# NeurAI-Lab/biHomE

Hardware: AMD Instinct MI355X
Metric: training image-pairs/s (128x128 patch, bs=64 per GPU, full step: fwd+bwd+Adam) (higher is better)
Workload: dtype f32

## Files before the change

bihome_amd/_lib.py:

```python
import ctypes
import os
from ctypes import POINTER, Structure, c_char_p, c_float, c_int, c_int64, c_void_p

_HERE = os.path.dirname(os.path.abspath(__file__))
TUNING = os.environ.get("BIHOME_TUNING") == "1"
_VARIANT = os.environ.get("BIHOME_LIB_VARIANT", "")
LIB_PATH = os.path.join(_HERE, "libbihome_hip_tuning.so" if TUNING else
                        ("libbihome_hip_%s.so" % _VARIANT if _VARIANT.isalnum() else "libbihome_hip.so"))


class BhConvDesc(Structure):
    _fields_ = [(n, c_int) for n in ("N", "Hi", "Wi", "Ci", "Ho", "Wo", "Co", "kh", "kw", "stride", "pad",
                                     "transposed", "in_nchw", "out_nchw", "precision", "w_layout", "route")] + \
               [("a_bound", c_void_p), ("b_bound", c_void_p)]


GEOMETRY_FIELDS = tuple(n for n, _ in BhConvDesc._fields_[:17])
AMAX_FLOATS = 512


class BhPack3x3Job(Structure):
    _fields_ = [("w", c_void_p), ("pf", c_void_p), ("pd", c_void_p), ("Co", c_int), ("Ci", c_int), ("split", c_int),
                ("reserved", c_int)]

# ... 117 lines not shown
        except AttributeError as e:
            raise BihomeLibError("bihome_amd: %s does not export %s (stale build?)" % (LIB_PATH, name)) from e
        fn.argtypes = argtypes
        fn.restype = c_int
    lib.bh_conv_wgrad_det_bytes.argtypes = [POINTER(BhConvDesc)]
    lib.bh_conv_wgrad_det_bytes.restype = c_int64
    lib.bh_stem7_wgrad_ws_bytes.argtypes = [POINTER(BhConvDesc)]
    lib.bh_stem7_wgrad_ws_bytes.restype = ctypes.c_size_t
    lib.bh_warp_bwd_img_scratch_doubles.argtypes = [c_int, c_int, c_int, c_int, c_int]
    lib.bh_warp_bwd_img_scratch_doubles.restype = ctypes.c_size_t
    if TUNING:
        lib.bh_debug_force_tile.argtypes = [c_int, c_int]
        lib.bh_debug_force_tile.restype = c_int
    return lib


lib = _load()
ROUTE_DETERMINISTIC, BN_DETERMINISTIC, F_DETERMINISTIC = 128, 32, 1
DSAC_METHODS = {"repr_error": 0, "inliers_ratio": 1, "soft_inliers_ratio": 2}
ROUTE_C3_PC = 512
ROUTE_WX3_PC = 1024
ROUTE_WX3_SHARED = 2048
ROUTE_GEMM_X3 = 4096
ROUTE_C3_TILE_WG = 256


def check(rc, what):
    if rc != 0:
        kind = {-1: "BH_E_BADARG", -2: "BH_E_UNSUPPORTED"}.get(rc, "hipError_t %d" % rc)
        raise BihomeLibError("%s failed: %s" % (what, kind))
```

bihome_amd/csrc/bn.hip:

```cpp
#include "common.h"

#define BN_MAX_CHUNKS 256

struct BnGeom {
    int groups, rows, C, C4, LPR, RPP, nchunks, rows_per_chunk;
    int det;
};

static bool bn_geom(int groups, int rows, int C, BnGeom& g, int det) {
    if (C % 4 || groups < 1 || rows < 1) return false;
    g.groups = groups; g.rows = rows; g.C = C; g.C4 = C / 4; g.det = det;
    if (g.C4 > 256 || (256 % g.C4)) return false;
    g.LPR = g.C4; g.RPP = 256 / g.LPR;
    int n = rows / (g.RPP * 4);
    if (n < 1) n = 1;
    if (n > BN_MAX_CHUNKS) n = BN_MAX_CHUNKS;
    g.rows_per_chunk = (rows + n - 1) / n;
    g.nchunks = (rows + g.rows_per_chunk - 1) / g.rows_per_chunk;
    return true;
}

template <int NV>
__device__ __forceinline__ void reduce_rows(double (&v)[NV], int LPR, int RPP, double* sm ) {
    for (int i = 0; i < NV; ++i) sm[threadIdx.x * NV + i] = v[i];
// ... 250 lines not shown
                                                           float* __restrict__ ggamma, float* __restrict__ gbeta,
                                                           unsigned* __restrict__ amax) {
    __shared__ float sm_amax[4];
    float vmax = 0.f;
    const int cq = threadIdx.x % g.LPR, r0 = threadIdx.x / g.LPR;
    const int grp = blockIdx.y;
    BnRaw raw[4];
    float4 cf4[4];
    double rs1[4], rs2[4];
#pragma unroll
    for (int i = 0; i < 4; ++i) {
        const int c = cq * 4 + i;
        cf4[i] = make_float4(0.f, 0.f, 0.f, 0.f); rs1[i] = 0; rs2[i] = 0;
        if (coef) {
            cf4[i] = coef[(size_t)grp * g.C + c];
            raw[i].gm = gamma ? gamma[c] : 1.f; raw[i].bt = beta ? beta[c] : 0.f; raw[i].s1 = 0; raw[i].s2 = 0;
        } else {
            raw[i] = bn_raw(stats, gamma, beta, nullptr, nullptr, 0, g.groups, grp, g.C, c, g.det);
            rs1[i] = bn_sum_total(sums, g.groups, grp, g.C, c, 0, g.det);
            rs2[i] = bn_sum_total(sums, g.groups, grp, g.C, c, 1, g.det);
        }
    }
    const size_t gbase = ((size_t)grp * g.rows) * g.C + cq * 4;
    const bool relu = flags & 1, mask_from_x = flags & 4;
    const bool rd_y = relu && !mask_from_x;
    const int stride = gridDim.x * g.RPP;
    int r = blockIdx.x * g.RPP + r0;
    float4 dv[4], av[4], yv[4];
    auto issue = [&](int rb) {
#pragma unroll
        for (int u = 0; u < 4; ++u) {
            const int rr = rb + u * stride;
            const size_t off = gbase + (size_t)rr * g.C;
            const bool ok = rr < g.rows;
            dv[u] = ok ? *reinterpret_cast<const float4*>(gy + off) : make_float4(0.f, 0.f, 0.f, 0.f);
            av[u] = ok ? *reinterpret_cast<const float4*>(x + off) : make_float4(0.f, 0.f, 0.f, 0.f);
            yv[u] = (ok && rd_y) ? *reinterpret_cast<const float4*>(y + off) : make_float4(0.f, 0.f, 0.f, 0.f);
        }
    };
    issue(r);
    float mean[4], invstd[4], sc[4], sh[4], k1[4], k2[4];
    const double inv_rows = 1.0 / (double)g.rows;
    const float invn = 1.0f / (float)g.rows;
#pragma unroll
    for (int i = 0; i < 4; ++i) {
        if (coef) {
            mean[i] = cf4[i].x; invstd[i] = cf4[i].y; k1[i] = cf4[i].z; k2[i] = cf4[i].w;
// ... 415 lines not shown
                       running_var, res, y, stats, g, eps, flags, use_running, momentum, upd ? running_mean : nullptr,
                       upd ? running_var : nullptr, reinterpret_cast<unsigned*>(amax_y));
    BH_LAUNCH_CHECK();
    return BH_OK;
}

int bh_bn_fwd_coeffs(const double* stats, const float* gamma, const float* beta, float* running_mean, float* running_var, int groups,
                     int rows, int C, float eps, float momentum, float* table, float* amax_y, void* stream) {
    BnGeom g;
    if (!stats || !table) return BH_E_BADARG;
    if (!bn_geom(groups, rows, C, g, -1)) return BH_E_UNSUPPORTED;
    const bool upd = running_mean && running_var;
    hipLaunchKernelGGL(bn_fwd_coeffs_kernel, dim3((groups * C + 255) / 256 + (upd ? 1 : 0)), dim3(256), 0, bh_stream(stream), stats, gamma, beta, g, eps,
                       momentum, upd ? running_mean : nullptr, upd ? running_var : nullptr, reinterpret_cast<float2*>(table),
                       reinterpret_cast<unsigned*>(amax_y));
    BH_LAUNCH_CHECK();
    return BH_OK;
}

int bh_bn_bwd(const float* gy, const float* y, const float* x, const float* gamma, const float* beta, const double* stats, float* gx,
              float* gres, float* ggamma, float* gbeta, double* scratch, int groups, int rows, int C, float eps, int flags,
              int use_running, const float* running_mean, const float* running_var, float* amax_gx, void* stream) {
    BnGeom g;
    if (!gy || !x || !gx || !stats || !scratch || ((flags & 1) && !(flags & 4) && !y)) return BH_E_BADARG;
    if ((flags & 4) && (flags & 2)) return BH_E_BADARG;
    if (C == 1) return amax_gx ? BH_E_UNSUPPORTED : bn1_bwd(gy, y, x, gamma, beta, stats, gx, gres, ggamma, gbeta, scratch, groups, rows, eps, flags, use_running,
                               running_mean, running_var, bh_stream(stream));
    if (!bn_geom(groups, rows, C, g, (flags & BH_BN_DETERMINISTIC) ? 1 : 0)) return BH_E_UNSUPPORTED;
    hipStream_t s = bh_stream(stream);
    if (flags & 16) {
        if (use_running) return BH_E_BADARG;
        hipLaunchKernelGGL(bn_bwd_apply_kernel, dim3(apply_blocks(g), groups), dim3(256), 0, s, gy, y, x, gamma, beta,
                           (const float4*)nullptr, gx, gres, g, flags, stats, (const double*)scratch, eps, ggamma, gbeta,
                           reinterpret_cast<unsigned*>(amax_gx));
        BH_LAUNCH_CHECK();
        return BH_OK;
    }
    float4* coef = reinterpret_cast<float4*>(scratch);
    double* part = scratch + (size_t)groups * C * 2;
    const bool need_sums = !use_running || ggamma || gbeta;
    if (need_sums) {
        hipLaunchKernelGGL(bn_bwd_reduce_kernel, dim3(g.nchunks, groups), dim3(256), 0, s, gy, y, x, gamma, beta, stats,
                           running_mean, running_var, g, eps, flags, use_running, part);
        BH_LAUNCH_CHECK();
    }
    BnGeom gf = g;
    if (!need_sums) gf.nchunks = 0;
    hipLaunchKernelGGL(bn_bwd_finalize_kernel, dim3(C), dim3(64), 0, s, part, gf, stats, running_mean, running_var, eps,
// ... 429 lines not shown
```

bihome_amd/csrc/conv3x3.hip:

```cpp
#include "common.h"
#include "conv3x3_args.h"
#include <type_traits>

#ifndef C3_X3_PIPE
#define C3_X3_PIPE 0
#endif

#ifndef C3_BN32_WAVES
#define C3_BN32_WAVES 2
#endif

#ifdef BH_TUNING
__device__ unsigned long long g_c3_ts[8 * 16384];
#define C3_STAMP(tile, k) do { if (a.dbg_ts && threadIdx.x == 0 && (tile) < 16384) { g_c3_ts[(tile) * 8 + (k)] = wall_clock64();          \
        if ((k) == 1 || (k) == 2) g_c3_ts[(tile) * 8 + 4 + (k)] = __builtin_readcyclecounter(); } } while (0)
#else
#define C3_STAMP(tile, k) do { } while (0)
#endif

constexpr int C3_HALO_BYTES = 8 * 200 * 16;
constexpr int C3_B_BYTES = 8192;
constexpr int C3_LDS_BYTES = 2 * C3_HALO_BYTES + 2 * C3_B_BYTES;

template <int BN, int SUBT, int TM, bool MAP4 = false>
// ... 77 lines not shown
#pragma unroll
                        for (int r = 0; r < 16; ++r)
                            zin[i][r] = __builtin_bit_cast(float, __builtin_amdgcn_raw_buffer_load_b32(rsZ, rowoff[r >> 2], C3_SOFF(i, r), 0));
                }
                if constexpr (ZM == 2) {
                    const __amdgpu_buffer_rsrc_t rsY = __builtin_amdgcn_make_buffer_rsrc(const_cast<float*>(a.bnr_y), 0, a.out_bytes, 0x00020000);
#pragma unroll
                    for (int i = 0; i < TM; ++i)
#pragma unroll
                        for (int r = 0; r < 16; ++r)
                            yin[i][r] = __builtin_bit_cast(float, __builtin_amdgcn_raw_buffer_load_b32(rsY, rowoff[r >> 2], C3_SOFF(i, r), 0));
                }
#pragma unroll
                for (int i = 0; i < TM; ++i)
#pragma unroll
                    for (int rq = 0; rq < 4; ++rq) {
                        float q1 = 0.f, q2 = 0.f;
#pragma unroll
                        for (int c = 0; c < 4; ++c) {
                            const int r = rq * 4 + c;
                            float v = acc[i][r] + bv;
                            if constexpr (HAS_EXTRA) v += ext[i][r];
                            if (a.relu) v = fmaxf(v, 0.0f);
                            __builtin_amdgcn_raw_buffer_store_b32(__builtin_bit_cast(unsigned, v), rsO, rowoff[rq], C3_SOFF(i, r), 0);
                            if constexpr (ZM > 0) {
                                const float zv = zin[i][r];
                                if (a.bnr_relu) {
                                    const float yv = ZM == 2 ? yin[i][r] : __builtin_fmaf(zv, r_sc, r_sh);
                                    if (!(yv > 0.f)) v = 0.f;
                                }
                                q1 += v; q2 = __builtin_fmaf(v, __builtin_fmaf(zv, r_invstd, c_x0), q2);
                            } else {
                                q1 += v; q2 = __builtin_fmaf(v, v, q2);
                            }
                        }
                        s1 += (double)q1; s2 += (double)q2;
                    }
            };
            using T_ = std::true_type; using F_ = std::false_type;
            using Z0 = std::integral_constant<int, 0>; using Z1 = std::integral_constant<int, 1>; using Z2 = std::integral_constant<int, 2>;
            if (rd_old || rd_res) {
                if (!rd_z) body(T_{}, Z0{}); else if (!rd_y) body(T_{}, Z1{}); else body(T_{}, Z2{});
            } else {
                if (!rd_z) body(F_{}, Z0{}); else if (!rd_y) body(F_{}, Z1{}); else body(F_{}, Z2{});
            }
        }
#undef C3_SOFF
    }
}

template <int BN, int PHASE>
__device__ __forceinline__ void c3_stats_merge(const C3Args& a, char* redb, double s1, double s2, int img, int g, int bx, int n0, int wave,
                                               int lane, int tid) {
    const int l31 = lane & 31, kh2 = lane >> 5;
    double* red = reinterpret_cast<double*>(redb);
// ... 552 lines not shown
                      d->Co % 64 == 0 && d->Ci % 64 == 0 && !bni && (!bn_sums || (groups >= 1 && d->N % groups == 0 && (d->N / groups) % 4 == 0));
    if (!map4 && (d->Hi % 8 || d->Wi % 8 || d->Ho != d->Hi || d->Wo != d->Wi)) return d->w_layout ? BH_E_UNSUPPORTED : 0;
    const int Kc = dgrad ? d->Co : d->Ci, Nn = dgrad ? d->Ci : d->Co;
    if (Kc % 32 || Nn % 32) return d->w_layout ? BH_E_UNSUPPORTED : 0;
    const int bn_tile = (Nn % 64) ? 32 : 64;
    const bool packed = d->w_layout != 0;
    const bool x3 = d->w_layout >= 2 && d->w_layout <= 4;
    const int np = d->w_layout >= 3 ? 2 : 3;
    const bool f16 = d->w_layout == 4;
    const bool bf16 = d->precision == 1;
    const long long src_bytes = (long long)d->N * d->Hi * d->Wi * Kc * 4, w_bytes = (long long)d->Co * 9 * d->Ci * (x3 ? 2 * np : 4);
    const long long out_bytes = (long long)d->N * d->Hi * d->Wi * Nn * 4;
    if (src_bytes >= (1ll << 31) || w_bytes >= (1ll << 31) || out_bytes >= (1ll << 31)) return 0;
    C3Args a = {};
    a.Src = src; a.Wt = w; a.bias = bias; a.Out = out;
    a.N = d->N; a.H = d->Hi; a.W = d->Wi; a.Kc = Kc; a.Nn = Nn; a.Cw = d->Ci; a.accumulate = accumulate;
    a.amax_src = reinterpret_cast<const unsigned*>(d->a_bound);
    a.src_bytes = (unsigned)src_bytes; a.w_bytes = (unsigned)w_bytes; a.out_bytes = (unsigned)out_bytes;
    if (bn_sums && (groups < 1 || d->N % groups || (!dgrad && bnr) || (dgrad && !bnr && accumulate))) return BH_E_BADARG;
    if (bnr) {
        if (!bnr->z || !bnr->stats) return BH_E_BADARG;
        a.bnr_z = bnr->z; a.bnr_y = bnr->y; a.bnr_stats = bnr->stats; a.bnr_gamma = bnr->gamma; a.bnr_beta = bnr->beta;
        a.bnr_eps = bnr->eps; a.bnr_relu = bnr->relu; a.bnr_rows = (d->N / groups) * d->Hi * d->Wi;
    }
    a.res = res; a.relu = relu; a.dbg_nch = g_c3_dbg_nch;
    a.bn_sums = bn_sums; a.imgs_per_group = bn_sums ? d->N / groups : 1; a.groups = groups;
    a.tiles_x = d->Wi / 8; a.tiles_per_img = (d->Hi / 8) * a.tiles_x; a.subtiles = d->N * a.tiles_per_img;
    if (map4) { a.tiles_x = 1; a.tiles_per_img = 1; a.subtiles = d->N / 4; }
    a.tx_shift = a.tpi_shift = -1;
    for (int b = 0; b < 24; ++b) {
        if (a.tiles_x == (1 << b)) a.tx_shift = b;
        if (a.tiles_per_img == (1 << b)) a.tpi_shift = b;
    }
    if (a.tx_shift < 0 || a.tpi_shift < 0) a.tx_shift = a.tpi_shift = -1;
    const bool few = (long long)((a.subtiles + 1) / 2) * (Nn / bn_tile) <= 256;
    const int subt = map4 ? 1 : (bn_tile == 64 && (g_c3_subt == 1 || (d->route & BH_ROUTE_C3_ONE_SUBTILE) || (g_c3_subt == 2 && few))) ? 1 : 2;
    dim3 grid((a.subtiles + subt - 1) / subt, Nn / bn_tile);
    a.gx_total = (int)grid.x; a.tpb = 1;
    {
        const long long wgs = (long long)grid.x * grid.y;
        if (g_c3_tpb >= 2 && !(d->route & BH_ROUTE_C3_ONE_POSITION) && subt == 2 && Kc / 32 > 1 && wgs > 512 && wgs <= 1024) {
            a.tpb = 2; grid.x = (grid.x + 1) / 2;
        }
    }
    if (bn_sums && !map4 && !(d->route & BH_ROUTE_C3_ONE_POSITION) && groups >= 1 && a.subtiles % (subt * groups) == 0) {
        const int ppg = a.subtiles / (subt * groups);
// ... 193 lines not shown
```

bihome_amd/csrc/conv3x3_args.h:

```cpp
#pragma once
#include "common.h"

typedef float f32x16 __attribute__((ext_vector_type(16)));
typedef float f32x8v __attribute__((ext_vector_type(8)));
typedef __bf16 bf16x8 __attribute__((ext_vector_type(8)));
typedef _Float16 f16x8 __attribute__((ext_vector_type(8)));
typedef __attribute__((address_space(3))) void* lds_void_ptr;

template <bool F16>
__device__ __forceinline__ f32x16 c3_mfma16(const uint4& av, const uint4& bv, const f32x16& c) {
    if constexpr (F16) return __builtin_amdgcn_mfma_f32_32x32x16_f16(__builtin_bit_cast(f16x8, av), __builtin_bit_cast(f16x8, bv), c, 0, 0, 0);
    else return __builtin_amdgcn_mfma_f32_32x32x16_bf16(__builtin_bit_cast(bf16x8, av), __builtin_bit_cast(bf16x8, bv), c, 0, 0, 0);
}

__device__ __forceinline__ bf16x8 c3_pack_bf16(const float4& lo, const float4& hi) {
    f32x8v v = {lo.x, lo.y, lo.z, lo.w, hi.x, hi.y, hi.z, hi.w};
    return __builtin_convertvector(v, bf16x8);
}

__device__ __forceinline__ int c3_strip_row(int q) { return q ^ (((q >> 1) ^ (q >> 2)) & 1); }

struct C3Args {
    const float* Src;
    const float* Wt;
    const float* bias;
    float* Out;
    int N, H, W;
    int Kc, Nn;
    int Cw;
    int accumulate;
    unsigned src_bytes, w_bytes, out_bytes;
    int tx_shift, tpi_shift;
    int tiles_x, tiles_per_img, subtiles;
    const float* res;
    int relu;
    const float* bnr_z;
    const float* bnr_y;
    const double* bnr_stats;
    const float* bnr_gamma;
    const float* bnr_beta;
    float bnr_eps;
    int bnr_relu, bnr_rows;
    double* bn_sums;
    int imgs_per_group, groups;
    int dbg_nch;
    int tpb, gx_total;
    int desync;
    int stat_acc;
    int NW;
    const float* bni;
    int bni_relu, bni_ipg, bni_groups, bni_lds;
    int dbg_noload;
    int dbg_ts;
    int det;
    const unsigned* amax_src;
};


int bh_conv3x3_pc_launch(C3Args& a, int dgrad, const float* bni_table, int bni_groups, int bni_relu, bool force, hipStream_t stream);
```

bihome_amd/csrc/conv3x3_pc.hip:

```cpp
#include "conv3x3_args.h"
#include <type_traits>

namespace {
constexpr int PC_HPL = 200;
constexpr int PC_PS = PC_HPL * 16 + 32;
constexpr int PC_PIECE = 4 * PC_PS;
constexpr int PC_STAGE = 2 * PC_PIECE;
constexpr int PC_BTAP = 8192;
constexpr int PC_BROW = 3 * PC_BTAP;
constexpr int PC_OFF_B = 2 * PC_STAGE;
constexpr int PC_OFF_EPI = PC_OFF_B + 3 * PC_BROW;
constexpr int PC_EPI_BYTES = 128 * 64 * 4;
constexpr int PC_OFF_RED = PC_OFF_EPI + PC_EPI_BYTES;
constexpr int PC_RED_BYTES = 4 * 128 * 8;
constexpr int PC_LDS = PC_OFF_RED + PC_RED_BYTES;
constexpr unsigned PC_XOOB = 0x80000000u;

#ifdef BH_TUNING
__device__ unsigned long long g_pc_ts[12 * 160 * 2];
#define PC_BARRIER()                                                                                                    \
    do {                                                                                                                \
        const bool st_ = a.dbg_ts && blockIdx.x == (unsigned)(a.dbg_ts - 1) && (tid & 63) == 0;                        \
        if (st_ && pc_nb < 160) g_pc_ts[(wave * 160 + pc_nb) * 2] = __builtin_readcyclecounter();                       \
        asm volatile("s_waitcnt lgkmcnt(0)\n\ts_barrier" ::: "memory");                                                \
// ... 449 lines not shown
        auto epi_fetch = [&](auto Q, int idx) {
            constexpr int q = decltype(Q)::value;
            if (nld == 0 || !((idx >> 2) ? fvalid[1] : fvalid[0])) return;
            const unsigned so = ((idx >> 2) ? fbase[1] : fbase[0]) + (unsigned)(idx & 3) * rowstep2;
            if constexpr (use_ext) pf_a[q] = __builtin_bit_cast(float4, __builtin_amdgcn_raw_buffer_load_b128(rsA_, voff, so, 0));
            if constexpr (rd_z) pf_z[q] = __builtin_bit_cast(float4, __builtin_amdgcn_raw_buffer_load_b128(rsZ, voff, so, 0));
            if constexpr (rd_y) pf_y[q] = __builtin_bit_cast(float4, __builtin_amdgcn_raw_buffer_load_b128(rsY, voff, so, 0));
        };
        int kout = 0;
        auto epi_run = [&](auto Q, int idx) {
            constexpr int q = decltype(Q)::value;
            if (!((idx >> 2) ? tvalid[1] : tvalid[0])) return;
            const unsigned so = ((idx >> 2) ? tbase[1] : tbase[0]) + (unsigned)(idx & 3) * rowstep2;
            const float4 av = *reinterpret_cast<const float4*>(epi_l + idx * 4096);
            const float4 z0 = make_float4(0.f, 0.f, 0.f, 0.f);
            const float4 o = use_ext ? pf_a[q] : z0, zz = rd_z ? pf_z[q] : z0, yy = rd_y ? pf_y[q] : z0;
            const float accv[4] = {av.x, av.y, av.z, av.w}, bb[4] = {bv.x, bv.y, bv.z, bv.w};
            const float oo[4] = {o.x, o.y, o.z, o.w};
            const float z4[4] = {zz.x, zz.y, zz.z, zz.w}, y4[4] = {yy.x, yy.y, yy.z, yy.w};
            const float isd[4] = {r_invstd.x, r_invstd.y, r_invstd.z, r_invstd.w}, cx[4] = {r_cx0.x, r_cx0.y, r_cx0.z, r_cx0.w};
            const float sc[4] = {r_sc.x, r_sc.y, r_sc.z, r_sc.w}, sh[4] = {r_sh.x, r_sh.y, r_sh.z, r_sh.w};
            float out[4];
            const bool do_relu = a.relu != 0, mask_on = rd_z && a.bnr_relu;
#pragma unroll
            for (int e = 0; e < 4; ++e) {
                float v = __builtin_ldexpf(accv[e], kout) + bb[e];
                if constexpr (use_ext) v += oo[e];
                v = do_relu ? fmaxf(v, 0.0f) : v;
                out[e] = v;
                if constexpr (stats) {
                    float vm = v, t = v;
                    if constexpr (rd_z) {
                        const float yv = rd_y ? y4[e] : __builtin_fmaf(z4[e], sc[e], sh[e]);
                        vm = (mask_on && !(yv > 0.f)) ? 0.f : v;
                        t = __builtin_fmaf(z4[e], isd[e], cx[e]);
                    }
                    S1[e] += (double)vm;
                    S2[e] = __builtin_fma((double)vm, (double)t, S2[e]);
                }
            }
            const __attribute__((ext_vector_type(4))) unsigned ov =
                __builtin_bit_cast(__attribute__((ext_vector_type(4))) unsigned, make_float4(out[0], out[1], out[2], out[3]));
            __builtin_amdgcn_raw_buffer_store_b128(ov, rsO, voff, so, 0);
            asm volatile("s_nop 3" :: "v"(ov));
            have = true;
        };
        using Q0 = std::integral_constant<int, 0>; using Q1 = std::integral_constant<int, 1>; using Q2 = std::integral_constant<int, 2>;
        using Q3 = std::integral_constant<int, 3>;
        const int nph = 3 * nch;
        const int grp = ew >> 1;
        const int nA = grp ? (nph - 1) / 2 : nph / 2;
        constexpr int UB = 4, NB = 2;
        const int BPP = (NB + nA - 1) / nA;
        auto run_batch = [&](int b) {
            const int i0 = b * UB;
            epi_run(Q0{}, i0 + 0); epi_run(Q1{}, i0 + 1); epi_run(Q2{}, i0 + 2); epi_run(Q3{}, i0 + 3);
        };
        auto fetch_batch = [&](int b) {
// ... 99 lines not shown
```

bihome_amd/kernels.py:

```python
import ctypes
import os

import torch

from ._lib import (AMAX_FLOATS, BN_DETERMINISTIC, DSAC_METHODS, F_DETERMINISTIC, GEOMETRY_FIELDS, ROUTE_DETERMINISTIC, ROUTE_WX3_PC, ROUTE_WX3_SHARED, BhBnIn, BhBnReduce, BhConvDesc,
                   BhPack3x3Job, check, lib)


def _p(t):
    return None if t is None else ctypes.c_void_p(t.data_ptr())


_DET_DEFAULT = os.environ.get("BIHOME_DETERMINISTIC", "0") == "1"
_DET_SCOPE = []


def set_deterministic(on=True):
    global _DET_DEFAULT
    prev, _DET_DEFAULT = _DET_DEFAULT, bool(on)
    return prev


def deterministic():
    return _DET_SCOPE[-1] if _DET_SCOPE else _DET_DEFAULT


class det_scope:

# ... 841 lines not shown


def conv_dgrad(gy, w, d, out=None, bn_reduce=None, wkey=None, wpacked=None, colsum=None, warp_sink=None):
    _chk(gy); _chk(w)
    _mark(d)
    if wpacked is not None:
        d, w = _route_det(getattr(d, "bh_packed", None) or _with_layout(d, packed_layout(d.precision))), wpacked
        if d.precision == F16X2:
            d.a_bound = amax_of(gy).data_ptr()
    if colsum is not None:
        assert out is None and bn_reduce is None
        _chk(colsum, torch.float64)
        out = torch.empty((d.N, d.Hi, d.Wi, d.Ci), dtype=torch.float32, device=gy.device)
        with _Timed(_conv_variant(d, "dgrad_colsum"), conv_flops(d), 4.0 * (gy.numel() + out.numel() + w.numel())):
            check(lib.bh_conv_dgrad_colsum(_p(gy), _p(w), _p(out), ctypes.byref(d), _p(colsum), _stream()), "bh_conv_dgrad_colsum")
        return out
    if bn_reduce is not None:
        acc = out is not None
        if out is None:
            out = torch.empty((d.N, d.Hi, d.Wi, d.Ci), dtype=torch.float32, device=gy.device)
        b = bn_reduce
        _chk(b["z"]); _chk(b["y"]); _chk(b["stats"], torch.float64); _chk(b["sums"], torch.float64)
        st = BhBnReduce(_p(b["z"]), _p(b["y"]), _p(b["stats"]), _p(b["gamma"]), _p(b["beta"]), float(b["eps"]), int(bool(b["relu"])))
        with _Timed(_conv_variant(d, "dgrad_bnr_y" if b["y"] is not None else "dgrad_bnr_z", acc, int(b["groups"])), conv_flops(d),
                    4.0 * (gy.numel() + out.numel() * ((3 if acc else 2) + (1 if b["y"] is not None else 0)) + w.numel())):
            check(lib.bh_conv_dgrad_bnreduce(_p(gy), _p(w), _p(out), ctypes.byref(d), int(acc), ctypes.byref(st), _p(b["sums"]),
                                             int(b["groups"]), _stream()), "bh_conv_dgrad_bnreduce")
        if acc:
            out._bh_amax = None
        return out
    if (out is None and not d.transposed and d.kh == 7 and d.stride == 2 and not d.out_nchw
            and (d.Ci == 1 or (d.Ci == 3 and d.in_nchw)) and d.Co % 4 == 0 and d.N * d.Ho * d.Wo >= 4096):
        if (d.Ci == 1 and d.Co == 64 and d.pad == 3 and d.Ho % 8 == 0 and d.Wo % 8 == 0 and d.Ho * 2 == d.Hi and d.Wo * 2 == d.Wi
                and w.is_contiguous() and os.environ.get("BIHOME_STEM_DGRAD_FUSED", "1") != "0"):
            if warp_sink is not None and not deterministic() and os.environ.get("BIHOME_WARP_IN_STEM_DGRAD", "1") != "0":
                ws_ = warp_sink
                _chk(ws_["src"]); _chk(ws_["H64"], torch.float64); _chk(ws_["gH"], torch.float64); _chk(ws_["g_cov"])
                with _Timed("stem7_dgrad_c1_kernel<true>", conv_flops(d), 4.0 * (gy.numel() + ws_["src"].numel())):
                    check(lib.bh_stem7_dgrad_c1_warp(_p(gy), _p(w), None, ctypes.byref(d), _p(ws_["src"]), _p(ws_["H64"]), _p(ws_["g_cov"]),
                                                     int(ws_["pool"]), _p(ws_["gH"]), _stream()), "bh_stem7_dgrad_c1_warp")
                ws_["done"] = True
                return None
            gx = torch.empty((d.N, d.Hi, d.Wi, 1), dtype=torch.float32, device=gy.device)
            with _Timed("stem7_dgrad_c1_kernel", conv_flops(d), 4.0 * (gy.numel() + gx.numel())):
                check(lib.bh_stem7_dgrad_c1(_p(gy), _p(w), _p(gx), ctypes.byref(d), _stream()), "bh_stem7_dgrad_c1")
            return gx
# ... 104 lines not shown
def bn_stats_buffer(groups, C, device):
    return torch.zeros(lib.bh_bn_stats_doubles(groups, C), dtype=torch.float64, device=device)


def bn_fwd(x, gamma, beta, rmean, rvar, res, groups, eps, momentum, relu, training, stats=None, stats_ready=False, amax=None):
    _chk(x); _chk(res)
    C = gamma.numel() if gamma is not None else x.shape[-1]
    rows = x.numel() // C // groups
    y = torch.empty_like(x)
    if stats is None:
        stats = bn_stats_buffer(groups, C, x.device)
        stats_ready = False
    flags = (1 if relu else 0) | (2 if res is not None else 0) | (8 if stats_ready else 0) | (BN_DETERMINISTIC if deterministic() else 0)
    nb = 4.0 * x.numel() * ((2 if (training and not stats_ready) else 1) + 1 + (1 if res is not None else 0))
    with _Timed("bn_fwd(%d kernels)" % (2 if (training and not stats_ready) else 1) + (" g%d rows%d C%d" % (groups, rows, C) if TIMING_DETAIL else ""), 0.0, nb):
        check(lib.bh_bn_fwd(_p(x), _p(gamma), _p(beta), _p(rmean), _p(rvar), _p(res), _p(y), _p(stats), groups, rows, C,
                            float(eps), float(momentum), flags, 0 if training else 1, _p(amax), _stream()), "bh_bn_fwd")
    if amax is not None:
        y._bh_amax = amax
    return y, stats


def bn_bwd(gy, y, x, gamma, stats, rmean, rvar, groups, eps, relu, training, want_gres, ggamma=None, gbeta=None, beta=None,
           had_res=None, scratch=None, sums_ready=None, amax=None):
    _chk(gy); _chk(x)
    C = gamma.numel() if gamma is not None else x.shape[-1]
    rows = x.numel() // C // groups
    gx = torch.empty_like(x)
    gres = torch.empty_like(x) if want_gres else None
    if sums_ready is not None:
        scratch = sums_ready
    elif scratch is None:
        scratch = torch.empty(lib.bh_bn_scratch_doubles(groups, C), dtype=torch.float64, device=x.device)
    had_res = want_gres if had_res is None else had_res
    mask_from_x = relu and not had_res
    flags = ((1 if relu else 0) | (2 if want_gres else 0) | (4 if mask_from_x else 0) | (16 if sums_ready is not None else 0)
             | (BN_DETERMINISTIC if deterministic() else 0))
    passes = 1 if sums_ready is not None else 2
    nb = 4.0 * x.numel() * (passes * (2 + (1 if (relu and not mask_from_x) else 0)) + 1 + (1 if want_gres else 0))
    with _Timed("bn_bwd(%d kernels)" % (1 if sums_ready is not None else 3) + (" g%d rows%d C%d" % (groups, rows, C) if TIMING_DETAIL else ""), 0.0, nb):
        check(lib.bh_bn_bwd(_p(gy), _p(y), _p(x), _p(gamma), _p(beta), _p(stats), _p(gx), _p(gres), _p(ggamma), _p(gbeta),
                            _p(scratch), groups, rows, C, float(eps), flags, 0 if training else 1, _p(rmean), _p(rvar),
                            _p(amax), _stream()), "bh_bn_bwd")
    if amax is not None:
        gx._bh_amax = amax
    return gx, gres


def bn_stats(x, stats, groups, C):
    _chk(x); _chk(stats, torch.float64)
    rows = x.numel() // C // groups
    with _Timed("bn_stats_kernel", 0.0, 4.0 * x.numel()):
        check(lib.bh_bn_stats(_p(x), _p(stats), groups, rows, C, BN_DETERMINISTIC if deterministic() else 0, _stream()), "bh_bn_stats")
    return stats


class BnPooled:
    __slots__ = ("pooled", "idx", "shape")

    def __init__(self, pooled, idx, shape):
        self.pooled, self.idx, self.shape = pooled, idx, tuple(shape)


def bn_maxpool_fwd(x, gamma, beta, rmean, rvar, groups, eps, momentum, relu, training, stats, stats_ready, want_index=True, amax=None):
    _chk(x)
    N, Hi, Wi, C = x.shape
    y = torch.empty((N, (Hi - 1) // 2 + 1, (Wi - 1) // 2 + 1, C), dtype=torch.float32, device=x.device)
    idx = torch.empty(y.shape, dtype=torch.uint8, device=x.device) if want_index else None
    flags = (1 if relu else 0) | (8 if stats_ready else 0) | (BN_DETERMINISTIC if deterministic() else 0)
# ... 189 lines not shown
```

bihome_amd/net.py:

```python
import os
import weakref

import torch
import torch.nn as nn

from . import kernels as K
from . import plan as P


def to_kernel_layout_(module):
    for m in module.modules():
        if isinstance(m, (nn.Conv2d, nn.ConvTranspose2d)):
            if not m.weight.data.is_contiguous(memory_format=torch.channels_last):
                m.weight.data = m.weight.data.contiguous(memory_format=torch.channels_last)
    return module


def kview(w):
    if w.dim() == 2:
        return w
    v = w.permute(0, 2, 3, 1)
    if not v.is_contiguous():
        raise RuntimeError("conv weight is not in kernel (channels_last) layout; call net.to_kernel_layout_(module)")
    return v
# ... 475 lines not shown
            K.conv_wgrad(x, g, gw, gb, d, det_ws=ws if d.bh_wx3 else None)
    _params_ready(s, m.weight, m.bias if has_gb else None)


def _bw_conv(s, i, op, g, x, need_src_grad):
    ctx, plan, grads = s.ctx, s.plan, s.grads
    d, wk = ctx.descs[i], ctx.weights[i]
    if op.relu:
        g = K.relu_bwd(g, s.slots[op.dst])
    if s.want_wgrad and op.mod.weight.requires_grad and op.extra["weight_fn"] is None:
        _enqueue_wgrad(s, i, op, g, x, d)
    if not need_src_grad:
        return
    if i in plan.from_1x1 and op.src not in grads:
        grads[op.src] = K.GradFrom1x1(g, wk)
        return
    red = None
    if i in plan.fuse_bn:
        b = plan.fuse_bn[i]
        bop, bm = s.prog.ops[b], s.prog.ops[b].mod
        sums = s.red_arena[plan.red_off[b]:plan.red_off[b] + K.bn_stats_doubles(ctx.groups, bm.num_features)]
        red = dict(z=s.slots[bop.src], y=s.slots[bop.dst] if (bop.relu and bop.res is not None) else None,
                   stats=ctx.stats[b], gamma=bm.weight, beta=bm.bias, eps=bm.eps, relu=bop.relu, sums=sums,
                   groups=ctx.groups)
        s.bn_reduced[b] = sums
    if i in plan.fuse_bias and op.src not in grads and red is None:
        p = plan.fuse_bias[i]
        grads[op.src] = K.conv_dgrad(g, wk, d, wpacked=ctx.wpacked.get(i),
                                     colsum=s.red_arena[plan.bias_off[p]:plan.bias_off[p] + K.bn_stats_doubles(1, d.Ci)])
    elif op.src in grads:
        K.conv_dgrad(g, wk, d, out=grads[op.src], bn_reduce=red, wkey=ctx.wkeys[i], wpacked=ctx.wpacked.get(i))
    else:
        gsrc = K.conv_dgrad(g, wk, d, bn_reduce=red, wkey=ctx.wkeys[i], wpacked=ctx.wpacked.get(i),
                            warp_sink=s.input_sink if (op.src == 0 and red is None) else None)
        if gsrc is not None:
            grads[op.src] = gsrc


def _bw_bn_join(s, i, op, g, x, need_src_grad):
    ctx, slots, amax_next = s.ctx, s.slots, s.amax_next
    j = ctx.joined[i]
    lop, m, lm = s.prog.ops[j], op.mod, s.prog.ops[j].mod
    train_a = s.want_wgrad and m.weight.requires_grad
    train_b = s.want_wgrad and lm.weight.requires_grad
    xb = slots[lop.src]
    gxa, gxb = K.bn_join_bwd(g, slots[op.dst], x, xb, m, lm, ctx.stats[i], ctx.stats[j], ctx.groups, op.relu, train_a, train_b,
                             amax_a=amax_next() if amax_next else None, amax_b=amax_next() if amax_next else None)
# ... 4 lines not shown
    if need_src_grad:
        _contribute(s.grads, op.src, gxa)
    if (lop.src != 0) or s.want_input_grad:
        _contribute(s.grads, lop.src, gxb)


def _bw_bn(s, i, op, g, x, need_src_grad):
    m, ctx, amax_next = op.mod, s.ctx, s.amax_next
    train_w = s.want_wgrad and m.weight is not None and m.weight.requires_grad
    ggamma, gbeta = (m.weight.grad, m.bias.grad) if train_w else (None, None)
    amax = amax_next() if (amax_next and m.num_features > 1) else None
    gres = None
    if isinstance(g, K.GradFrom1x1):
        gx = K.bn_bwd_from_1x1(g, x, m.weight, m.bias, ctx.stats[i], ctx.groups, m.eps, op.relu, ggamma, gbeta, amax=amax)
    elif isinstance(g, K.PooledGrad):
        gx = K.bn_maxpool_bwd(g, x, m.weight, m.bias, ctx.stats[i], m.running_mean, m.running_var, ctx.groups, m.eps, op.relu,
                              ctx.training, ggamma, gbeta, amax=amax)
    else:
        yb = s.slots[op.dst]
        if isinstance(yb, (K.BnOnLoad, K.BnPooled)):
            yb = None
        gx, gres = K.bn_bwd(g, yb, x, m.weight, ctx.stats[i], m.running_mean, m.running_var, ctx.groups,
                            m.eps, op.relu, ctx.training, op.res is not None and ((op.res != 0) or s.want_input_grad),
                            ggamma, gbeta, beta=m.bias, had_res=op.res is not None, sums_ready=s.bn_reduced.get(i), amax=amax)
    if train_w and s.on_param_grad is not None:
        s.on_param_grad(m.weight)
        s.on_param_grad(m.bias)
    if need_src_grad:
        _contribute(s.grads, op.src, gx)
    if gres is not None:
        _contribute(s.grads, op.res, gres)


def _bw_tail(s, i, op, g, x, need_src_grad):
    ctx = s.ctx
    c1, bn, c2 = op.mod
    tr = s.want_wgrad and c1.weight.requires_grad
    N, h, w, _ = x.shape
    eval_b1 = tr and not ctx.training and c1.bias is not None and c1.bias.requires_grad
    gbeta0 = bn.bias.grad.clone() if eval_b1 else None
    gx = K.tail_bwd(g, x, kview(c1.weight), c1.bias, bn.weight, bn.bias, kview(c2.weight), ctx.stats[i],
                    bn.running_mean, bn.running_var, ctx.groups, h * w, bn.eps, ctx.training, need_src_grad,
                    kview(c1.weight.grad) if tr else None, bn.weight.grad if tr else None,
                    bn.bias.grad if tr else None, kview(c2.weight.grad) if tr else None,
                    c2.bias.grad if (tr and c2.bias is not None) else None)
    if eval_b1:
        with torch.no_grad():
# ... 208 lines not shown
```

bihome_amd/plan.py:

```python
import torch.nn as nn

from . import kernels as K


class ProgramIndex:
    __slots__ = ("nops", "producer", "consumers", "users", "consumer", "last_consumer")

    def __init__(self, ops):
        self.nops = len(ops)
        self.producer = {op.dst: j for j, op in enumerate(ops)}
        self.consumers = {}
        self.consumer = {}
        for j, op in enumerate(ops):
            self.consumers.setdefault(op.src, []).append(j)
            if op.res is not None:
                self.consumers.setdefault(op.res, []).append(j)
            self.consumer.setdefault(op.src, j)
        self.users = {s: len(v) for s, v in self.consumers.items()}
        self.last_consumer = {s: v[0] for s, v in self.consumers.items()}


def packs_weight(op, device=None):
    m = op.mod
    return (op.kind == "conv" and isinstance(m, nn.Conv2d) and op.extra["weight_fn"] is None and m.kernel_size == (3, 3)
# ... 119 lines not shown
    p.folded = plan_folded(prog, ix, fold)
    p.deferred = set(p.folded.values())
    p.bn_off, p.total, p.nrec = plan_forward_arenas(prog, groups, precision)
    return p


def forward_plan(prog, training, groups, precision, packer, fold):
    key = forward_key(prog, training, groups, precision, packer, fold)
    p = prog.fw_plans.get(key)
    if p is None:
        if len(prog.fw_plans) > 16:
            prog.fw_plans.clear()
        p = prog.fw_plans[key] = make_forward_plan(prog, training, groups, precision,
                                                   set(packer.entries) if packer is not None else None, fold)
    assert p.nops == len(prog.ops), "Program grew after it first ran"
    prog.last_forward_plan = p
    return p


FROM_1X1_KC = (16,)


class BackwardPlan:
    __slots__ = ("nops", "consumed_by", "fuse_bn", "fuse_bias", "from_1x1", "red_off", "bias_off", "total", "nrec")


def backward_key(prog, ctx, gout_shape, want_wgrad):
    return (bool(ctx.training), bool(want_wgrad), int(ctx.groups), tuple(gout_shape), frozenset(ctx.joined.items()), frozenset(ctx.descs),
            ctx.precision,
            tuple((op.mod.weight.requires_grad, op.mod.bias is not None and op.mod.bias.requires_grad) for op in prog.ops if op.kind == "conv"))


def plan_fuse_bn(prog, ix, ctx):
    fuse_bn = {}
    if ctx.training:
        ops, descs = prog.ops, ctx.descs
        for j, op in enumerate(ops):
            b = ix.producer.get(op.src)
            if (op.kind == "conv" and b is not None and ops[b].kind == "bn" and ix.last_consumer.get(op.src) == j
                    and j in descs and descs[j].bh_reduce_ok and descs[j].N % ctx.groups == 0 and b not in ctx.joined):
                fuse_bn[j] = b
    return fuse_bn


def plan_fuse_bias(prog, ix, ctx, want_wgrad, fuse_bn):
    fuse_bias = {}
    if want_wgrad:
        ops, descs = prog.ops, ctx.descs
        for j, op in enumerate(ops):
            p = ix.producer.get(op.src)
            if (op.kind == "conv" and j not in fuse_bn and p is not None and ops[p].kind == "conv" and ix.users.get(op.src, 0) == 1
                    and j in descs and p in descs and descs[j].bh_reduce_ok and not ops[p].relu):
                pm = ops[p].mod
                if pm.bias is not None and pm.bias.requires_grad and pm.weight.requires_grad and ops[p].extra["weight_fn"] is None:
                    fuse_bias[j] = p
    return fuse_bias


def plan_from_1x1(prog, ix, ctx, fuse_bn):
    from_1x1 = set()
    if ctx.training:
        ops = prog.ops
        for j, op in enumerate(ops):
            b = ix.producer.get(op.src)
            m = op.mod
# ... 4 lines not shown
                    and not op.extra["in_nchw"] and not op.extra["out_nchw"]):
                from_1x1.add(j)
    return from_1x1


def plan_backward_arenas(prog, ctx, fuse_bn, fuse_bias):
    red_off, bias_off, total = {}, {}, 0
    for j, p in fuse_bias.items():
        bias_off[p] = total
        total += K.bn_stats_doubles(1, ctx.descs[j].Ci)
    for b in fuse_bn.values():
        red_off[b] = total
        total += K.bn_stats_doubles(ctx.groups, prog.ops[b].mod.num_features)
    nrec = max(1, sum(1 for op in prog.ops if op.kind == "bn")) if ctx.precision == K.F16X2 else 0
    return red_off, bias_off, total, nrec


def make_backward_plan(prog, ctx, want_wgrad):
    ix = prog.index()
    p = BackwardPlan()
    p.nops = ix.nops
    p.consumed_by = ix.users
    p.fuse_bn = plan_fuse_bn(prog, ix, ctx)
    p.fuse_bias = plan_fuse_bias(prog, ix, ctx, want_wgrad, p.fuse_bn)
    p.from_1x1 = plan_from_1x1(prog, ix, ctx, p.fuse_bn)
    p.red_off, p.bias_off, p.total, p.nrec = plan_backward_arenas(prog, ctx, p.fuse_bn, p.fuse_bias)
    return p


def backward_plan(prog, ctx, gout_shape, want_wgrad):
    key = backward_key(prog, ctx, gout_shape, want_wgrad)
    p = prog.bw_plans.get(key)
    if p is None:
        p = prog.bw_plans[key] = make_backward_plan(prog, ctx, want_wgrad)
    assert p.nops == len(prog.ops), "Program grew after it first ran"
    prog.last_backward_plan = p
    return p
```

include/bihome.h:

```cpp
#ifndef BIHOME_H
#define BIHOME_H

#include <stdint.h>

#ifdef __cplusplus
extern "C" {
#endif

#define BH_OK 0
#define BH_E_BADARG (-1)
#define BH_E_UNSUPPORTED (-2)

int bh_version(void);
int bh_device_arch(char* buf, int buflen);

#define BH_F_DETERMINISTIC 1
#define BH_BN_DETERMINISTIC 32
int bh_probe_mfma_bf16(int random_operands, float* sink_dev, double* tflops, void* stream);
int bh_probe_mfma_f32(int random_operands, float* sink_dev, double* tflops, void* stream);


int bh_h4pt_fwd(const float* delta, int B, float W, float H, double* H64, float* H32, void* stream);
int bh_h4pt_bwd(const float* delta, const double* H64, const double* gH, int B, float W, float H,
                float* gdelta, void* stream);
// ... 92 lines not shown
    int in_nchw;
    int out_nchw;
    int precision;
    int w_layout;
    int route;
    const float* a_bound;
    const float* b_bound;
} bh_conv_desc;
#define BH_AMAX_FLOATS 512
int bh_absmax(const float* x, long long n, float* record, void* stream);
#define BH_ROUTE_GENERIC_CONV 1
#define BH_ROUTE_HALO_SMALL 2
#define BH_ROUTE_NO_STEM7 4
#define BH_ROUTE_WGRAD_GENERIC 8
#define BH_ROUTE_WGRAD_3TAP 16
#define BH_ROUTE_C3_ONE_SUBTILE 32
#define BH_ROUTE_C3_ONE_POSITION 64
#define BH_ROUTE_DETERMINISTIC 128
#define BH_ROUTE_C3_PC 512
#define BH_ROUTE_C3_TILE_WG 256
#define BH_ROUTE_WX3_PC 1024
#define BH_ROUTE_WX3_SHARED 2048
#define BH_ROUTE_GEMM_X3 4096

typedef struct {
    const float* w;
    float* pf;
    float* pd;
    int Co, Ci;
    int split;
    int reserved;
} bh_pack3x3_job;
int bh_conv3x3_pack(const bh_pack3x3_job* jobs_dev, int njobs, void* stream);
int bh_conv3x3_pack_f16(const bh_pack3x3_job* jobs_dev, int njobs, void* stream);

int bh_conv_variant(const bh_conv_desc* d, int which, int accumulate, int bn_groups, char* buf, int n);

#ifdef BH_TUNING
int bh_debug_force_tile(int bm, int bn);
#endif
int bh_conv_fwd(const float* x, const float* w, const float* bias, float* y, const bh_conv_desc* d, void* stream);
int bh_conv_fwd_amax(const float* x, const float* w, const float* bias, float* y, const bh_conv_desc* d, float* amax_y, void* stream);

int bh_conv_fwd_act(const float* x, const float* w, const float* bias, const float* res, float* y, const bh_conv_desc* d,
                    int relu, void* stream);
typedef struct {
// ... 112 lines not shown
```

Before: 5158.

## Store ReLU-masked gradient from fused dgrad+BN-reduce to skip y reads and gres buffer

When a BN+ReLU with residual feeds a 3x3 conv whose dgrad is fused with the BN reduction, the dgrad epilogue now writes the ReLU-masked gradient instead of the raw one. The later BN backward apply kernel can then skip re-reading y for the mask, and the residual gradient reuses the masked gradient tensor instead of a separately allocated and written gres buffer. This cuts memory traffic and allocation in residual blocks. It relies on the planner's single-writer and last-consumer conditions so that overwriting the stored gradient with its masked form stays correct.

After: 5183, median of 6. Within noise of the previous version (+0.5%).

```diff
diff --git a/bihome_amd/_lib.py b/bihome_amd/_lib.py
--- a/bihome_amd/_lib.py
+++ b/bihome_amd/_lib.py
@@ -163,6 +163,8 @@
 ROUTE_WX3_PC = 1024
 ROUTE_WX3_SHARED = 2048
 ROUTE_GEMM_X3 = 4096
+ROUTE_BNR_STORE_MASKED = 8192
+BN_GRAD_MASKED = 64
 ROUTE_C3_TILE_WG = 256
 
 
diff --git a/bihome_amd/csrc/bn.hip b/bihome_amd/csrc/bn.hip
--- a/bihome_amd/csrc/bn.hip
+++ b/bihome_amd/csrc/bn.hip
@@ -296,7 +296,7 @@
         }
     }
     const size_t gbase = ((size_t)grp * g.rows) * g.C + cq * 4;
-    const bool relu = flags & 1, mask_from_x = flags & 4;
+    const bool relu = (flags & 1) && !(flags & 64), mask_from_x = flags & 4;
     const bool rd_y = relu && !mask_from_x;
     const int stride = gridDim.x * g.RPP;
     int r = blockIdx.x * g.RPP + r0;
@@ -758,8 +758,9 @@
               float* gres, float* ggamma, float* gbeta, double* scratch, int groups, int rows, int C, float eps, int flags,
               int use_running, const float* running_mean, const float* running_var, float* amax_gx, void* stream) {
     BnGeom g;
-    if (!gy || !x || !gx || !stats || !scratch || ((flags & 1) && !(flags & 4) && !y)) return BH_E_BADARG;
+    if (!gy || !x || !gx || !stats || !scratch || ((flags & 1) && !(flags & (4 | 64)) && !y)) return BH_E_BADARG;
     if ((flags & 4) && (flags & 2)) return BH_E_BADARG;
+    if ((flags & 64) && (!(flags & 16) || !(flags & 1) || gres || C == 1)) return BH_E_BADARG;
     if (C == 1) return amax_gx ? BH_E_UNSUPPORTED : bn1_bwd(gy, y, x, gamma, beta, stats, gx, gres, ggamma, gbeta, scratch, groups, rows, eps, flags, use_running,
                                running_mean, running_var, bh_stream(stream));
     if (!bn_geom(groups, rows, C, g, (flags & BH_BN_DETERMINISTIC) ? 1 : 0)) return BH_E_UNSUPPORTED;
diff --git a/bihome_amd/csrc/conv3x3.hip b/bihome_amd/csrc/conv3x3.hip
--- a/bihome_amd/csrc/conv3x3.hip
+++ b/bihome_amd/csrc/conv3x3.hip
@@ -123,15 +123,16 @@
                             float v = acc[i][r] + bv;
                             if constexpr (HAS_EXTRA) v += ext[i][r];
                             if (a.relu) v = fmaxf(v, 0.0f);
-                            __builtin_amdgcn_raw_buffer_store_b32(__builtin_bit_cast(unsigned, v), rsO, rowoff[rq], C3_SOFF(i, r), 0);
                             if constexpr (ZM > 0) {
-                                const float zv = zin[i][r];
+                                const float gv = v, zv = zin[i][r];
                                 if (a.bnr_relu) {
                                     const float yv = ZM == 2 ? yin[i][r] : __builtin_fmaf(zv, r_sc, r_sh);
                                     if (!(yv > 0.f)) v = 0.f;
                                 }
+                                __builtin_amdgcn_raw_buffer_store_b32(__builtin_bit_cast(unsigned, a.bnr_store_masked ? v : gv), rsO, rowoff[rq], C3_SOFF(i, r), 0);
                                 q1 += v; q2 = __builtin_fmaf(v, __builtin_fmaf(zv, r_invstd, c_x0), q2);
                             } else {
+                                __builtin_amdgcn_raw_buffer_store_b32(__builtin_bit_cast(unsigned, v), rsO, rowoff[rq], C3_SOFF(i, r), 0);
                                 q1 += v; q2 = __builtin_fmaf(v, v, q2);
                             }
                         }
@@ -730,6 +731,7 @@
         if (!bnr->z || !bnr->stats) return BH_E_BADARG;
         a.bnr_z = bnr->z; a.bnr_y = bnr->y; a.bnr_stats = bnr->stats; a.bnr_gamma = bnr->gamma; a.bnr_beta = bnr->beta;
         a.bnr_eps = bnr->eps; a.bnr_relu = bnr->relu; a.bnr_rows = (d->N / groups) * d->Hi * d->Wi;
+        a.bnr_store_masked = (bnr->relu && (d->route & BH_ROUTE_BNR_STORE_MASKED)) ? 1 : 0;
     }
     a.res = res; a.relu = relu; a.dbg_nch = g_c3_dbg_nch;
     a.bn_sums = bn_sums; a.imgs_per_group = bn_sums ? d->N / groups : 1; a.groups = groups;
diff --git a/bihome_amd/csrc/conv3x3_args.h b/bihome_amd/csrc/conv3x3_args.h
--- a/bihome_amd/csrc/conv3x3_args.h
+++ b/bihome_amd/csrc/conv3x3_args.h
@@ -41,6 +41,7 @@
     const float* bnr_beta;
     float bnr_eps;
     int bnr_relu, bnr_rows;
+    int bnr_store_masked;
     double* bn_sums;
     int imgs_per_group, groups;
     int dbg_nch;
diff --git a/bihome_amd/csrc/conv3x3_pc.hip b/bihome_amd/csrc/conv3x3_pc.hip
--- a/bihome_amd/csrc/conv3x3_pc.hip
+++ b/bihome_amd/csrc/conv3x3_pc.hip
@@ -495,6 +495,7 @@
             const float sc[4] = {r_sc.x, r_sc.y, r_sc.z, r_sc.w}, sh[4] = {r_sh.x, r_sh.y, r_sh.z, r_sh.w};
             float out[4];
             const bool do_relu = a.relu != 0, mask_on = rd_z && a.bnr_relu;
+            const bool store_masked = stats && rd_z && a.bnr_store_masked;
 #pragma unroll
             for (int e = 0; e < 4; ++e) {
                 float v = __builtin_ldexpf(accv[e], kout) + bb[e];
@@ -507,6 +508,7 @@
                         const float yv = rd_y ? y4[e] : __builtin_fmaf(z4[e], sc[e], sh[e]);
                         vm = (mask_on && !(yv > 0.f)) ? 0.f : v;
                         t = __builtin_fmaf(z4[e], isd[e], cx[e]);
+                        if (store_masked) out[e] = vm;
                     }
                     S1[e] += (double)vm;
                     S2[e] = __builtin_fma((double)vm, (double)t, S2[e]);
diff --git a/bihome_amd/kernels.py b/bihome_amd/kernels.py
--- a/bihome_amd/kernels.py
+++ b/bihome_amd/kernels.py
@@ -3,7 +3,7 @@
 
 import torch
 
-from ._lib import (AMAX_FLOATS, BN_DETERMINISTIC, DSAC_METHODS, F_DETERMINISTIC, GEOMETRY_FIELDS, ROUTE_DETERMINISTIC, ROUTE_WX3_PC, ROUTE_WX3_SHARED, BhBnIn, BhBnReduce, BhConvDesc,
+from ._lib import (AMAX_FLOATS, BN_DETERMINISTIC, BN_GRAD_MASKED, ROUTE_BNR_STORE_MASKED, DSAC_METHODS, F_DETERMINISTIC, GEOMETRY_FIELDS, ROUTE_DETERMINISTIC, ROUTE_WX3_PC, ROUTE_WX3_SHARED, BhBnIn, BhBnReduce, BhConvDesc,
                    BhPack3x3Job, check, lib)
 
 
@@ -891,6 +891,8 @@
         b = bn_reduce
         _chk(b["z"]); _chk(b["y"]); _chk(b["stats"], torch.float64); _chk(b["sums"], torch.float64)
         st = BhBnReduce(_p(b["z"]), _p(b["y"]), _p(b["stats"]), _p(b["gamma"]), _p(b["beta"]), float(b["eps"]), int(bool(b["relu"])))
+        masked = bool(b.get("store_masked")) and bool(b["relu"])
+        d.route = (d.route | ROUTE_BNR_STORE_MASKED) if masked else (d.route & ~ROUTE_BNR_STORE_MASKED)
         with _Timed(_conv_variant(d, "dgrad_bnr_y" if b["y"] is not None else "dgrad_bnr_z", acc, int(b["groups"])), conv_flops(d),
                     4.0 * (gy.numel() + out.numel() * ((3 if acc else 2) + (1 if b["y"] is not None else 0)) + w.numel())):
             check(lib.bh_conv_dgrad_bnreduce(_p(gy), _p(w), _p(out), ctypes.byref(d), int(acc), ctypes.byref(st), _p(b["sums"]),
@@ -1041,12 +1043,14 @@
 
 
 def bn_bwd(gy, y, x, gamma, stats, rmean, rvar, groups, eps, relu, training, want_gres, ggamma=None, gbeta=None, beta=None,
-           had_res=None, scratch=None, sums_ready=None, amax=None):
+           had_res=None, scratch=None, sums_ready=None, amax=None, grad_masked=False):
     _chk(gy); _chk(x)
     C = gamma.numel() if gamma is not None else x.shape[-1]
     rows = x.numel() // C // groups
+    if grad_masked:
+        assert sums_ready is not None and relu and training, "grad_masked: only behind conv_dgrad(bn_reduce=dict(store_masked=True, relu=True))"
     gx = torch.empty_like(x)
-    gres = torch.empty_like(x) if want_gres else None
+    gres = torch.empty_like(x) if (want_gres and not grad_masked) else None
     if sums_ready is not None:
         scratch = sums_ready
     elif scratch is None:
@@ -1054,16 +1058,16 @@
     had_res = want_gres if had_res is None else had_res
     mask_from_x = relu and not had_res
     flags = ((1 if relu else 0) | (2 if want_gres else 0) | (4 if mask_from_x else 0) | (16 if sums_ready is not None else 0)
-             | (BN_DETERMINISTIC if deterministic() else 0))
+             | (BN_GRAD_MASKED if grad_masked else 0) | (BN_DETERMINISTIC if deterministic() else 0))
     passes = 1 if sums_ready is not None else 2
-    nb = 4.0 * x.numel() * (passes * (2 + (1 if (relu and not mask_from_x) else 0)) + 1 + (1 if want_gres else 0))
+    nb = 4.0 * x.numel() * (passes * (2 + (1 if (relu and not mask_from_x and not grad_masked) else 0)) + 1 + (1 if gres is not None else 0))
     with _Timed("bn_bwd(%d kernels)" % (1 if sums_ready is not None else 3) + (" g%d rows%d C%d" % (groups, rows, C) if TIMING_DETAIL else ""), 0.0, nb):
         check(lib.bh_bn_bwd(_p(gy), _p(y), _p(x), _p(gamma), _p(beta), _p(stats), _p(gx), _p(gres), _p(ggamma), _p(gbeta),
                             _p(scratch), groups, rows, C, float(eps), flags, 0 if training else 1, _p(rmean), _p(rvar),
                             _p(amax), _stream()), "bh_bn_bwd")
     if amax is not None:
         gx._bh_amax = amax
-    return gx, gres
+    return gx, (gy if (want_gres and grad_masked) else gres)
 
 
 def bn_stats(x, stats, groups, C):
diff --git a/bihome_amd/net.py b/bihome_amd/net.py
--- a/bihome_amd/net.py
+++ b/bihome_amd/net.py
@@ -521,7 +521,7 @@
         sums = s.red_arena[plan.red_off[b]:plan.red_off[b] + K.bn_stats_doubles(ctx.groups, bm.num_features)]
         red = dict(z=s.slots[bop.src], y=s.slots[bop.dst] if (bop.relu and bop.res is not None) else None,
                    stats=ctx.stats[b], gamma=bm.weight, beta=bm.bias, eps=bm.eps, relu=bop.relu, sums=sums,
-                   groups=ctx.groups)
+                   groups=ctx.groups, store_masked=b in plan.masked_store)
         s.bn_reduced[b] = sums
     if i in plan.fuse_bias and op.src not in grads and red is None:
         p = plan.fuse_bias[i]
@@ -572,7 +572,8 @@
             yb = None
         gx, gres = K.bn_bwd(g, yb, x, m.weight, ctx.stats[i], m.running_mean, m.running_var, ctx.groups,
                             m.eps, op.relu, ctx.training, op.res is not None and ((op.res != 0) or s.want_input_grad),
-                            ggamma, gbeta, beta=m.bias, had_res=op.res is not None, sums_ready=s.bn_reduced.get(i), amax=amax)
+                            ggamma, gbeta, beta=m.bias, had_res=op.res is not None, sums_ready=s.bn_reduced.get(i), amax=amax,
+                            grad_masked=i in s.bn_reduced and i in s.plan.masked_store)
     if train_w and s.on_param_grad is not None:
         s.on_param_grad(m.weight)
         s.on_param_grad(m.bias)
diff --git a/bihome_amd/plan.py b/bihome_amd/plan.py
--- a/bihome_amd/plan.py
+++ b/bihome_amd/plan.py
@@ -165,12 +165,12 @@
 
 
 class BackwardPlan:
-    __slots__ = ("nops", "consumed_by", "fuse_bn", "fuse_bias", "from_1x1", "red_off", "bias_off", "total", "nrec")
+    __slots__ = ("nops", "consumed_by", "fuse_bn", "masked_store", "fuse_bias", "from_1x1", "red_off", "bias_off", "total", "nrec")
 
 
 def backward_key(prog, ctx, gout_shape, want_wgrad):
     return (bool(ctx.training), bool(want_wgrad), int(ctx.groups), tuple(gout_shape), frozenset(ctx.joined.items()), frozenset(ctx.descs),
-            ctx.precision,
+            ctx.precision, bool(MASKED_STORE),
             tuple((op.mod.weight.requires_grad, op.mod.bias is not None and op.mod.bias.requires_grad) for op in prog.ops if op.kind == "conv"))
 
 
@@ -184,6 +184,26 @@
                     and j in descs and descs[j].bh_reduce_ok and descs[j].N % ctx.groups == 0 and b not in ctx.joined):
                 fuse_bn[j] = b
     return fuse_bn
+
+
+MASKED_STORE = True
+
+
+def plan_masked_store(prog, ix, fuse_bn, enabled=None):
+    if enabled is None:
+        enabled = MASKED_STORE
+    marked = set()
+    if enabled:
+        ops = prog.ops
+        writers = {}
+        for op in ops:
+            writers[op.dst] = writers.get(op.dst, 0) + 1
+        for j, b in fuse_bn.items():
+            bop = ops[b]
+            if (bop.kind == "bn" and bop.relu and bop.res is not None and ops[j].src == bop.dst
+                    and ix.last_consumer.get(bop.dst) == j and writers.get(bop.dst, 0) == 1):
+                marked.add(b)
+    return marked
 
 
 def plan_fuse_bias(prog, ix, ctx, want_wgrad, fuse_bn):
@@ -234,6 +254,7 @@
     p.nops = ix.nops
     p.consumed_by = ix.users
     p.fuse_bn = plan_fuse_bn(prog, ix, ctx)
+    p.masked_store = plan_masked_store(prog, ix, p.fuse_bn)
     p.fuse_bias = plan_fuse_bias(prog, ix, ctx, want_wgrad, p.fuse_bn)
     p.from_1x1 = plan_from_1x1(prog, ix, ctx, p.fuse_bn)
     p.red_off, p.bias_off, p.total, p.nrec = plan_backward_arenas(prog, ctx, p.fuse_bn, p.fuse_bias)
diff --git a/include/bihome.h b/include/bihome.h
--- a/include/bihome.h
+++ b/include/bihome.h
@@ -138,6 +138,7 @@
 #define BH_ROUTE_WX3_PC 1024
 #define BH_ROUTE_WX3_SHARED 2048
 #define BH_ROUTE_GEMM_X3 4096
+#define BH_ROUTE_BNR_STORE_MASKED 8192
 
 typedef struct {
     const float* w;
```
